# artpixls/ART

Measured on AMD Instinct MI355X. Metric: megapixels/sec end-to-end (AMaZE+FTblockDN+tone), 45 MP Bayer, higher is better.
Workload: dtype f32; 1 GPU; AMaZE + getImage/matrix + ImProcFunctions::denoise (chroma noise-curve map, FTblockDN wavelet shrinkage luma 40 / chroma 15 / gamma 1.7 + DCT detail recovery 50) + exposure 0.3 EV + tone curve STD, 8192x5464 Bayer RGGB fp32, 1 frame per GPU per step (BASELINE configs[2]); frame=8192x5464, lanes_per_gpu=1, parallelism=frame-per-gpu x1, completion_records=1, completion_via=single process

## Files before the change

### art_amd/csrc/artgpu_api.hip

```cpp
#include <hip/hip_runtime.h>
#include <dlfcn.h>
#include <cmath>
#include <cstdio>
#include <cstdarg>
#include <cstring>
#include <new>
#include <string>
#include <thread>
#include <vector>
#include <algorithm>

#include "../../include/artgpu.h"
#include "kernels.h"

using namespace artgpu;

struct artgpu_ctx {
    int device = 0;
    hipStream_t stream = nullptr;
    hipStream_t aux = nullptr;
    hipEvent_t aux_ev[2] = {nullptr, nullptr};
    hipStream_t dn_stream[1] = {nullptr};
    hipEvent_t dn_ev[2] = {nullptr, nullptr};
    const float *gam_tab = nullptr; float gam_key[6] = {};
    int opt_lut_lds = 1;
    int opt_dn_streams = 0;
    int ccalc_nonneg = 0;
    int opt_dn_fused = 1;
    std::string err;
    int *fs_diag = nullptr;
    int opt_dn_debug_stall = -1;
    long opt_dn_wait_ms = 0;
    long long batch_px = 0;
    int dn_form = -1, dn_form_streak = 0;
    float *arena = nullptr;
    size_t arena_bytes = 0;
    static constexpr int NSTAGE = 8;
    float *stage[NSTAGE] = {};
    size_t stage_bytes[NSTAGE] = {};
    static constexpr int NPOOL = 64;
    float *pool[NPOOL] = {};
    size_t pool_bytes[NPOOL] = {};
    std::vector<artgpu_ctx *> lanes;
    int batch_lanes = 1;
    int frames_in_flight = 1;
    bool owns_stream = false;
    hipStream_t io_up = nullptr, io_down = nullptr;
    hipEvent_t io_ev[8] = {};
    int *io_host = nullptr;
    int io_host_cap = 0;
// ... 375 lines not shown
        const size_t nfixed = (((size_t)ctx->amz_nstream + (1 + ctx->amz_narena) + (1 + ctx->amz_narena + ctx->amz_nstream) + 3) / 4) * 4;
        int v = 0;
        HIPCHK(ctx, hipMemcpy(&v, reinterpret_cast<int *>(ctx->amz_lists) + nfixed + 4 + 2 * (size_t)ctx->amz_nstream + (n[13] - '0'), sizeof(int), hipMemcpyDeviceToHost));
        *value = v;
        return ARTGPU_OK;
    }
    return fail(ctx, ARTGPU_EINVAL, "get_option: unknown option '%s'", name);
}

int artgpu_set_option(artgpu_ctx *ctx, const char *name, long value)
{
    if (!ctx || !name) return ARTGPU_EINVAL;
    const std::string n(name);
    if (n == "amaze_path") { if (value < 0 || value > 1) return fail(ctx, ARTGPU_EINVAL, "amaze_path: 0 or 1"); ctx->opt_amaze_path = (int)value; }
    else if (n == "amaze_split") ctx->opt_amaze_split = value != 0;
    else if (n == "amaze_overlap") ctx->opt_amaze_overlap = value != 0;
    else if (n == "amaze_grid") { if (value < 0) return fail(ctx, ARTGPU_EINVAL, "amaze_grid: >= 0"); ctx->opt_amaze_grid = (int)value; }
    else if (n == "amaze_zero_mask") ctx->opt_amaze_zero_mask = value;
    else if (n == "amaze_zero_frame") ctx->opt_amaze_zero_frame = (int)value;
    else if (n == "amaze_poison") ctx->opt_amaze_poison = (int)value;
    else if (n == "roctx") ctx->opt_roctx = value != 0;
    else if (n == "dn_streams") ctx->opt_dn_streams = value != 0;
    else if (n == "dn_fused") ctx->opt_dn_fused = (int)value;
    else if (n == "dn_debug_stall") ctx->opt_dn_debug_stall = (int)value;
    else if (n == "dn_wait_ms") ctx->opt_dn_wait_ms = value < 0 ? 0 : value;
    else if (n == "lut_lds") ctx->opt_lut_lds = value != 0;
    else if (n == "cu_reserve") { if (value < 0 || value > 4096) return fail(ctx, ARTGPU_EINVAL, "cu_reserve: 0 .. 4096"); ctx->cu_reserve = (int)value; }
    else if (n == "io_direct") { if (value < -1 || value > 4096) return fail(ctx, ARTGPU_EINVAL, "io_direct: -1 (automatic), 0 .. 4096 workgroups"); ctx->opt_io_direct = (int)value; }
    else if (n == "rcd_rows") { if (value != 4 && value != 8) return fail(ctx, ARTGPU_EINVAL, "rcd_rows: 4 or 8"); ctx->opt_rcd_rows = (int)value; }
    else return fail(ctx, ARTGPU_EINVAL, "set_option: unknown option '%s'", name);
    return ARTGPU_OK;
}

int artgpu_set_progress_callback(artgpu_ctx *ctx, artgpu_progress_fn fn, void *user)
{
    if (!ctx) return ARTGPU_EINVAL;
    ctx->progress_fn = fn;
    ctx->progress_user = user;
    return ARTGPU_OK;
}

int artgpu_enable_timing(artgpu_ctx *ctx, int enable)
{
    if (!ctx) return ARTGPU_EINVAL;
    ctx->timing = enable != 0;
    return ARTGPU_OK;
// ... 391 lines not shown
    a.tail_kind = ctx->curve_tail_kind == ARTGPU_CURVE_TAIL_HOST ? 0 : ctx->curve_tail_kind; a.tail_y = ctx->curve_tail_y; a.tail_pc = ctx->curve_tail_pc;
    if (lut65536) {
        if ((rc = upload_curve(ctx, lut65536))) return rc;
        a.lut = ctx->lut;
    }
    a.no_lds_lut = !ctx->opt_lut_lds; a.cu_reserve = ctx->cu_reserve;
    HIPCHK(ctx, launch_tone_std(a, ctx->stream));
    return unbind_rgb(ctx, image, &d);
}

}

struct artgpu_wavelet {
    int w = 0, h = 0, w2 = 0, h2 = 0, nlevels = 0;
    float *bands = nullptr;
    float *lowpass[2] = {nullptr, nullptr};
    int cur = 0;
    size_t n = 0;
    float *band(int l, int dir) const { return bands + ((size_t)l * 3 + (dir - 1)) * n; }
};

namespace {
int wavelet_skip(int level) { return level <= 1 ? 1 : 1 << (level - 1); }
}

extern "C" {

int artgpu_wavelet_decompose(artgpu_ctx *ctx, const artgpu_plane *src, int maxlvl, artgpu_wavelet **out)
{
    if (!ctx) return ARTGPU_EINVAL;
    if (!plane_ok(src) || !out || maxlvl < 1 || maxlvl > 9) return fail(ctx, ARTGPU_EINVAL, "wavelet_decompose: bad arguments");
    *out = nullptr;
    const int w = src->w, h = src->h, w2 = (w + 1) / 2, h2 = (h + 1) / 2;
    if ((w2 < h2 ? w2 : h2) < 2 * wavelet_skip(maxlvl - 1) || w < 8 || h < 8)
        return fail(ctx, ARTGPU_EUNSUPPORTED, "wavelet_decompose: %dx%d too small for %d levels", w, h, maxlvl);
    HIPCHK(ctx, hipSetDevice(ctx->device));
    const float *dsrc = src->p;
    size_t sstride = (size_t)(src->row_stride_bytes / 4);
    if (!src->on_device) {
        int rc = ensure(ctx, &ctx->stage[0], &ctx->stage_bytes[0], (size_t)w * h * 4);
        if (rc) return rc;
        HIPCHK(ctx, hipMemcpy2DAsync(ctx->stage[0], (size_t)w * 4, src->p, (size_t)src->row_stride_bytes, (size_t)w * 4, h, hipMemcpyHostToDevice, ctx->stream));
        dsrc = ctx->stage[0];
        sstride = w;
    }
    artgpu_wavelet *wv = new (std::nothrow) artgpu_wavelet;
    if (!wv) return fail(ctx, ARTGPU_ENOMEM, "wavelet_decompose: out of host memory");
    wv->w = w; wv->h = h; wv->w2 = w2; wv->h2 = h2; wv->nlevels = maxlvl; wv->n = (size_t)w2 * h2;
    hipError_t e = hipMalloc(reinterpret_cast<void **>(&wv->bands), (size_t)maxlvl * 3 * wv->n * sizeof(float));
    if (e == hipSuccess) e = hipMalloc(reinterpret_cast<void **>(&wv->lowpass[0]), wv->n * sizeof(float));
    if (e == hipSuccess) e = hipMalloc(reinterpret_cast<void **>(&wv->lowpass[1]), wv->n * sizeof(float));
    if (e != hipSuccess) {
        artgpu_wavelet_free(ctx, wv);
        return fail(ctx, ARTGPU_ENOMEM, "wavelet_decompose: hipMalloc failed: %s", hipGetErrorString(e));
    }
    WaveArgs a = {};
    a.w = w; a.h = h; a.w2 = w2; a.h2 = h2;
    for (int l = 0; l < maxlvl; ++l) {
        a.b1 = wv->band(l, 1); a.b2 = wv->band(l, 2); a.b3 = wv->band(l, 3);
        hipError_t le;
        if (l == 0) {
            a.src = dsrc; a.src_stride = sstride; a.lo = wv->lowpass[0];
            wv->cur = 0;
            le = launch_wavelet_analysis0(a, ctx->stream);
        } else {
            a.src = wv->lowpass[wv->cur]; a.lo = wv->lowpass[wv->cur ^ 1]; a.skip = wavelet_skip(l);
            le = launch_wavelet_haar_analysis(a, ctx->stream);
            wv->cur ^= 1;
        }
        if (le != hipSuccess) {
            artgpu_wavelet_free(ctx, wv);
            return fail(ctx, ARTGPU_EHIP, "wavelet_decompose: launch failed: %s", hipGetErrorString(le));
        }
    }
    if (!src->on_device) {
        const hipError_t se = hipStreamSynchronize(ctx->stream);
        if (se != hipSuccess) {
            artgpu_wavelet_free(ctx, wv);
            return fail(ctx, ARTGPU_EHIP, "wavelet_decompose: %s", hipGetErrorString(se));
        }
    }
    *out = wv;
    return ARTGPU_OK;
}

int artgpu_wavelet_info(const artgpu_wavelet *wv, int32_t *w2, int32_t *h2, int32_t *nlevels)
{
    if (!wv) return ARTGPU_EINVAL;
    if (w2) *w2 = wv->w2;
    if (h2) *h2 = wv->h2;
    if (nlevels) *nlevels = wv->nlevels;
    return ARTGPU_OK;
}

int artgpu_wavelet_get_band(artgpu_ctx *ctx, const artgpu_wavelet *wv, int level, int dir, float *dst, int on_device)
{
// ... 13 lines not shown
    HIPCHK(ctx, hipSetDevice(ctx->device));
    float *p = dir == 0 ? wv->lowpass[wv->cur] : wv->band(level, dir);
    HIPCHK(ctx, hipMemcpyAsync(p, src, wv->n * sizeof(float), on_device ? hipMemcpyDeviceToDevice : hipMemcpyHostToDevice, ctx->stream));
    if (!on_device) HIPCHK(ctx, hipStreamSynchronize(ctx->stream));
    return ARTGPU_OK;
}

int artgpu_wavelet_reconstruct(artgpu_ctx *ctx, artgpu_wavelet *wv, artgpu_plane *dst, float blend)
{
    if (!ctx) return ARTGPU_EINVAL;
    if (!wv || !plane_ok(dst) || dst->w != wv->w || dst->h != wv->h) return fail(ctx, ARTGPU_EINVAL, "wavelet_reconstruct: bad arguments");
    HIPCHK(ctx, hipSetDevice(ctx->device));
    float *ddst = dst->p;
    size_t dstride = (size_t)(dst->row_stride_bytes / 4);
    if (!dst->on_device) {
        int rc = ensure(ctx, &ctx->stage[0], &ctx->stage_bytes[0], (size_t)wv->w * wv->h * 4);
        if (rc) return rc;
        HIPCHK(ctx, hipMemcpy2DAsync(ctx->stage[0], (size_t)wv->w * 4, dst->p, (size_t)dst->row_stride_bytes, (size_t)wv->w * 4, wv->h, hipMemcpyHostToDevice, ctx->stream));
        ddst = ctx->stage[0];
        dstride = wv->w;
    }
    WaveArgs a = {};
    a.w = wv->w; a.h = wv->h; a.w2 = wv->w2; a.h2 = wv->h2; a.blend = blend;
    for (int l = wv->nlevels - 1; l > 0; --l) {
        a.src = wv->lowpass[wv->cur]; a.lo = wv->lowpass[wv->cur ^ 1];
        a.b1 = wv->band(l, 1); a.b2 = wv->band(l, 2); a.b3 = wv->band(l, 3); a.skip = wavelet_skip(l);
        HIPCHK(ctx, launch_wavelet_haar_synthesis(a, ctx->stream));
        wv->cur ^= 1;
    }
    a.src = wv->lowpass[wv->cur];
    a.b1 = wv->band(0, 1); a.b2 = wv->band(0, 2); a.b3 = wv->band(0, 3);
    a.dst = ddst; a.dst_stride = dstride;
    HIPCHK(ctx, launch_wavelet_synthesis0(a, ctx->stream));
    if (!dst->on_device) {
        HIPCHK(ctx, hipMemcpy2DAsync(dst->p, (size_t)dst->row_stride_bytes, ddst, (size_t)wv->w * 4, (size_t)wv->w * 4, wv->h, hipMemcpyDeviceToHost, ctx->stream));
        HIPCHK(ctx, hipStreamSynchronize(ctx->stream));
    }
    return ARTGPU_OK;
}

int artgpu_wavelet_free(artgpu_ctx *ctx, artgpu_wavelet *wv)
{
    if (!wv) return ARTGPU_EINVAL;
    if (ctx) { (void)hipSetDevice(ctx->device); (void)hipStreamSynchronize(ctx->stream); }
    if (wv->bands) (void)hipFree(wv->bands);
    if (wv->lowpass[0]) (void)hipFree(wv->lowpass[0]);
    if (wv->lowpass[1]) (void)hipFree(wv->lowpass[1]);
    delete wv;
    return ARTGPU_OK;
}

}

namespace {

enum { P_L = 0, P_A, P_B, P_LBANDS, P_LLOW0, P_LLOW1, P_CBANDS, P_CLOW0, P_CLOW1, P_SF, P_TMP, P_HISTO, P_MAD, P_GAM, P_CCALC, P_LIN, P_BLOCKS, P_DTAB, P_CCMAP, P_CACHEF, P_PQ, P_XCBRT, P_GAUSS64, P_DMASK, P_LABTABS, P_PIPE_R, P_PIPE_G, P_PIPE_B, P_DNINFO, P_BATCH, P_DCTTAB, P_CBANDS2, P_CLOW0_2, P_CLOW1_2, P_SF_A, P_SF_B, P_HISTO_A, P_HISTO_B, P_RGBCURVES, P_FUSED, P_LBANDS2,
       P_IO_IN0, P_IO_IN1, P_IO_CFA, P_IO_IMG0, P_IO_IMG1, P_IO_IMG2, P_IO_IMG3, P_IO_IMG4, P_IO_IMG5, P_IO_OUT0, P_IO_OUT1, P_IO_FLAGS,
       P_NSLOTS };
static_assert(P_NSLOTS <= artgpu_ctx::NPOOL, "grow artgpu_ctx::pool");

struct DevDecomp {
    float *bands, *low[2];
    int cur, nlevels, w, h, w2, h2;
    size_t n;
    float *band(int l, int dir) const { return bands + ((size_t)l * 3 + (dir - 1)) * n; }
};

int decompose_dev(artgpu_ctx *ctx, DevDecomp &d, const float *src, hipStream_t st = nullptr)
{
    if (!st) st = ctx->stream;
    WaveArgs a = {};
    a.w = d.w; a.h = d.h; a.w2 = d.w2; a.h2 = d.h2;
    for (int l = 0; l < d.nlevels; ++l) {
        a.b1 = d.band(l, 1); a.b2 = d.band(l, 2); a.b3 = d.band(l, 3);
        if (l == 0) {
            a.src = src; a.src_stride = d.w; a.lo = d.low[0]; d.cur = 0;
            HIPCHK(ctx, launch_wavelet_analysis0(a, st));
        } else {
            a.src = d.low[d.cur]; a.lo = d.low[d.cur ^ 1]; a.skip = wavelet_skip(l);
            HIPCHK(ctx, launch_wavelet_haar_analysis(a, st));
            d.cur ^= 1;
        }
    }
    return ARTGPU_OK;
}

int reconstruct_dev(artgpu_ctx *ctx, DevDecomp &d, float *dst, hipStream_t st = nullptr)
{
    if (!st) st = ctx->stream;
    WaveArgs a = {};
    a.w = d.w; a.h = d.h; a.w2 = d.w2; a.h2 = d.h2; a.blend = 1.f;
    for (int l = d.nlevels - 1; l > 0; --l) {
        a.src = d.low[d.cur]; a.lo = d.low[d.cur ^ 1];
        a.b1 = d.band(l, 1); a.b2 = d.band(l, 2); a.b3 = d.band(l, 3); a.skip = wavelet_skip(l);
        HIPCHK(ctx, launch_wavelet_haar_synthesis(a, st));
        d.cur ^= 1;
    }
    a.src = d.low[d.cur];
    a.b1 = d.band(0, 1); a.b2 = d.band(0, 2); a.b3 = d.band(0, 3);
    a.dst = dst; a.dst_stride = d.w;
    HIPCHK(ctx, launch_wavelet_synthesis0(a, st));
    return ARTGPU_OK;
}

int pool_get(artgpu_ctx *ctx, int slot, size_t bytes, float **out)
{
    int rc = ensure(ctx, &ctx->pool[slot], &ctx->pool_bytes[slot], bytes);
    *out = ctx->pool[slot];
    return rc;
}

}

extern "C" {

namespace {
int detail_mask_dev(artgpu_ctx *ctx, const float *src, size_t src_stride, float *mask, int W, int H,
                    float scaling, float threshold, float ceiling, float factor, float blur, float *scratch);
}

int artgpu_wavelet_mad(artgpu_ctx *ctx, const artgpu_wavelet *wv, float *mad_sqr)
{
    if (!ctx) return ARTGPU_EINVAL;
    if (!wv || !mad_sqr) return fail(ctx, ARTGPU_EINVAL, "wavelet_mad: null argument");
    if (wv->n > 0x7fffffff) return fail(ctx, ARTGPU_EUNSUPPORTED, "wavelet_mad: band larger than an int holds (MadRgb's datalen is an int)");
// ... 166 lines not shown
    px.igam_lds_lo = 8000;
    if (lab_mode) {
        float *tabs;
        const bool fresh = ctx->pool[P_LABTABS] == nullptr;
        if ((rc = pool_get(ctx, P_LABTABS, 4 * 65536 * 4, &tabs))) return rc;
        if (fresh) {
            std::vector<float> host(4 * 65536);
            build_cachef(host.data()); build_cachefy(host.data() + 65536);
            build_denoise_gamma_tabs(host.data() + 2 * 65536, host.data() + 3 * 65536);
            hipError_t e = hipMemcpyAsync(tabs, host.data(), host.size() * 4, hipMemcpyHostToDevice, sL);
            if (e == hipSuccess) e = hipStreamSynchronize(sL);
            if (e != hipSuccess) {
                (void)hipFree(ctx->pool[P_LABTABS]); ctx->pool[P_LABTABS] = nullptr; ctx->pool_bytes[P_LABTABS] = 0;
                return fail(ctx, ARTGPU_EHIP, "rgb_denoise: upload of the Lab tables failed: %s", hipGetErrorString(e));
            }
        }
        px.lab_mode = 1;
        px.cachef = tabs; px.cachefy = tabs + 65536; px.dn_gamma = tabs + 2 * 65536; px.dn_igamma = tabs + 3 * 65536;
        for (int k = 0; k < 9; ++k) { px.wpi[k] = ws[k]; px.iws[k] = iws[k]; }
    }
    px.realred = realred; px.realblue = realblue; px.qhighFactor = aggressive ? 1.f / static_cast<float>(0.9) : 1.0f;
    HIPCHK(ctx, launch_rgb2yuv(px, sL));

    if ((rc = decompose_dev(ctx, Ld, L, sL))) return rc;
    if (!merged_mad) HIPCHK(ctx, launch_mad(Ld.bands, n2, nsub, reinterpret_cast<int *>(histo_fc[0]), madL, sL));

    auto fused_pass = [&](bool ab, const float *cin, float *cout, const float *cL, const float *mL, const float *mab, int lev0, int nb,
                          float nv_const, float noisevar_ab) -> int {
        FusedShrinkArgs fa = {};
        if (ab) { fa.coefC = cout; fa.nL = 0; fa.nsub_ch = nb; }
        else { fa.coef = cin; fa.coef_out = cout; fa.nL = nb; }
        fa.coefL = cL; fa.n = n2; fa.w = w2; fa.h = h2;
        fa.madL = mL; fa.madab = mab;
        fa.noisevar = ccalc_dev; fa.noisevar_nonneg = ctx->ccalc_nonneg; fa.noisevar_const = nv_const; fa.noisevar_scale = maxNoiseVarab; fa.noisevar_ab[0] = fa.noisevar_ab[1] = noisevar_ab;
        fa.useNoiseCCurve = useNoiseCCurve ? 1 : 0;
        for (int l = 0; l < 10; ++l) fa.rad[l] = bl0.rad[l];
        fa.level0 = lev0; fa.nsub = nb; fa.diag = ctx->fs_diag; fa.wait_ticks = (long long)ctx->opt_dn_wait_ms * 100000LL; fa.stall_band = ctx->opt_dn_debug_stall < 0 ? -1 : ctx->opt_dn_debug_stall >> 16; fa.stall_strip = ctx->opt_dn_debug_stall < 0 ? -1 : ctx->opt_dn_debug_stall & 0xffff;
        HIPCHK(ctx, launch_shrink_blur(fa, fused_scratch, sL));
        return ARTGPU_OK;
    };

    float noisevar_abc[2];
    auto chroma_front = [&](int ch) -> int {
        DevDecomp &Cd = Cdd[ch];
        float *sf = sfc[1 + ch], *tmp = tmpc[1 + ch], *madab = mad + 32 * (1 + ch);
        int *histo = reinterpret_cast<int *>(histo_fc[1 + ch]);
        float noisevar_ab = ch == 0 ? noisevarab_r : noisevarab_b;
        if (autoch && noisevar_ab <= 0.001f) noisevar_ab = 0.02f;
        noisevar_abc[ch] = noisevar_ab;
        int rc2;
        if ((rc2 = decompose_dev(ctx, Cd, ch == 0 ? A : B, sL))) return rc2;
        if (aggressive && noisevar_ab > 0.001f) {
            HIPCHK(ctx, launch_mad(Cd.bands, n2, nsub, histo, madab, sL));
            ShrinkArgs sa = {};
            sa.n = n2; sa.noisevar = ccalc_dev; sa.noisevar_scale = maxNoiseVarab; sa.noisevar_ab = noisevar_ab; sa.useNoiseCCurve = useNoiseCCurve ? 1 : 0;
            const size_t top = (size_t)(nsub - 3) * n2;
            sa.coef = Cd.bands + top; sa.coefL = Ld.bands + top; sa.sfave = sf; sa.madL = madL + (nsub - 3); sa.madab = madab + (nsub - 3);
            if (fused) {
                if ((rc2 = fused_pass(true, Cd.bands + top, Cd.bands + top, Ld.bands + top, madL + (nsub - 3), madab + (nsub - 3), levwav - 1, 3, 0.f, noisevar_ab))) return rc2;
            } else {
                HIPCHK(ctx, launch_shrink_sf(sa, 3, true, sL));
                BlurArgs bt = bl0;
                bt.level0 = levwav - 1;
                bt.src = sf; bt.dst = tmp;
                HIPCHK(ctx, launch_hblur(bt, 3, sL));
                bt.src = tmp; bt.sfave = sf; bt.coef = Cd.bands + top;
                HIPCHK(ctx, launch_vblur_combine(bt, 3, sL));
            }
            if (nsub > 3) {
                sa.coef = Cd.bands; sa.coefL = Ld.bands; sa.madL = madL; sa.madab = madab;
                HIPCHK(ctx, launch_bishrink_AB(sa, nsub - 3, sL));
            }
        }
        if (noisevar_ab > 0.001f && !merged_mad) {
// ... 22 lines not shown
                HIPCHK(ctx, launch_hblur(bl, nsub, sL));
                bl.src = tmp; bl.sfave = sf; bl.coef = Cd.bands;
                HIPCHK(ctx, launch_vblur_combine(bl, nsub, sL));
            }
        }
        if (nresi || highresi) {
            float host[32];
            HIPCHK(ctx, launch_mad(Cd.bands, n2, nsub, histo, madab, sL));
            HIPCHK(ctx, hipMemcpyAsync(host, madab, (size_t)nsub * sizeof(float), hipMemcpyDeviceToHost, sL));
            HIPCHK(ctx, hipStreamSynchronize(sL));
            float resid = 0.f, maxresid = 0.f;
            for (int k = 0; k < nsub; ++k) {
                resid += host[k];
                if (host[k] > maxresid) maxresid = host[k];
            }
            if (ch == 0) { chresidtemp = resid; chmaxresidtemp = maxresid; }
            else {
                float chresid = resid + chresidtemp, chmaxresid = maxresid + chmaxresidtemp;
                chresid = std::sqrt(chresid / (6 * (levwav)));
                if (highresi) *highresi = chresid + 0.66f * (std::sqrt(chmaxresid) - chresid);
                if (nresi) *nresi = chresid;
            }
        }
        return reconstruct_dev(ctx, Cd, ch == 0 ? A : B, sL);
    };

    float *Lout = L;
    auto luma = [&](hipStream_t sd) -> int {
        if (!denoiseLuminance) return ARTGPU_OK;
        int rc2;
        const int nsubL = 3 * (levwav < 5 ? levwav : 5);
        float *sf = sfc[0], *tmp = tmpc[0];
        BlurArgs bl = bl0;
        ShrinkArgs sa = {};
        sa.coef = Ld.bands; sa.sfave = sf; sa.n = n2; sa.madL = madL; sa.noisevar = nullptr; sa.noisevar_const = noisevarL;
        DevDecomp Lrec = Ld;
        if (merged) Lrec.bands = Lbands2;
        for (int rep = aggressive ? 0 : 1; rep < 2 && !merged; ++rep) {
            if (fused) {
                float *dstb = Lbands2 ? Lbands2 : Ld.bands;
                if ((rc2 = fused_pass(false, Lrec.bands, dstb, nullptr, madL, nullptr, 0, nsubL, noisevarL, 0.f))) return rc2;
                Lrec.bands = dstb;
            } else {
                HIPCHK(ctx, launch_shrink_sf(sa, nsubL, false, sL));
                bl.src = sf; bl.dst = tmp;
                HIPCHK(ctx, launch_hblur(bl, nsubL, sL));
                bl.src = tmp; bl.sfave = sf; bl.coef = Ld.bands;
                HIPCHK(ctx, launch_vblur_combine(bl, nsubL, sL));
            }
        }
        if (Lrec.bands != Ld.bands && nsubL < nsub)
            HIPCHK(ctx, hipMemcpyAsync(Lrec.bands + (size_t)nsubL * n2, Ld.bands + (size_t)nsubL * n2, (size_t)(nsub - nsubL) * n2 * 4, hipMemcpyDeviceToDevice, sL));
        if (do_detail) {
            if ((rc2 = pool_get(ctx, P_LIN, n * 4, &Lout))) return rc2;
        }
        Lrec.cur = Ld.cur;
        if ((rc2 = reconstruct_dev(ctx, Lrec, Lout, sL))) return rc2;
        if (do_detail) {
            float *Lin = L;
            DetailArgs da = {};
            da.w = w; da.h = h;
            da.numblox_W = (int)std::ceil(((float)w) / 25) + 2;
            da.numblox_H = (int)std::ceil(((float)h) / 25) + 2;
            const float params_Ldetail = std::min(float(p->luminance_detail), 99.9f);
            auto compute_detail = [](float dd) -> float { const float t = static_cast<float>((100. - dd) * (100. - dd) + 50. * (100. - dd)) * 64 * 0.5f; return t * t; };
            da.detail_hi = compute_detail(params_Ldetail);
            da.detail_lo = compute_detail(0.f);
            { const int br = int(3 / scale); da.blur_rad = br > 1 ? br : 1; }
            float *dtab;
            const bool fresh_dtab = ctx->pool[P_DCTTAB] == nullptr;
            if ((rc2 = pool_get(ctx, P_DCTTAB, 4 * 4096 * 4, &dtab))) return rc2;
            if ((rc2 = pool_get(ctx, P_BLOCKS, (size_t)da.numblox_W * da.numblox_H * 4096 * 4, &da.blocks))) return rc2;
            if (fresh_dtab) {
                std::vector<float> host(4 * 4096);
                float *tm_in = host.data(), *tm_out = tm_in + 4096, *ct = tm_out + 4096, *ctt = ct + 4096;
                const float epsilon = 0.001f / (64 * 64);
                const int border = 4;
                for (int i = 0; i < 64; ++i) {
                    const float i1 = std::abs((i > 32 ? i - 64 + 1 : i));
                    const float vmask = (i1 < border ? (float)0 + (std::sin((M_PI * i1) / (2 * border)) * std::sin((M_PI * i1) / (2 * border))) : 1.0f);
// ... 1398 lines not shown
        if (rc) return rc;
        c->batch_px = 0;
    }
    if (px > c->batch_px) c->batch_px = px;
    return ARTGPU_OK;
}

int batch_prepare_lanes(artgpu_ctx *ctx, int L)
{
    HIPCHK(ctx, hipSetDevice(ctx->device));
    while ((int)ctx->lanes.size() < L - 1) {
        artgpu_ctx *peer = nullptr;
        int rc = artgpu_create(ctx->device, &peer);
        if (rc) return fail(ctx, rc, "batch_run: cannot create lane %d", (int)ctx->lanes.size() + 1);
        if (hipStreamCreateWithFlags(&peer->stream, hipStreamNonBlocking) != hipSuccess) { (void)artgpu_destroy(peer); return fail(ctx, ARTGPU_EHIP, "batch_run: stream"); }
        peer->owns_stream = true;
        ctx->lanes.push_back(peer);
    }
    for (artgpu_ctx *peer : ctx->lanes) {
        peer->curve_tail_kind = ctx->curve_tail_kind; peer->curve_tail_y = ctx->curve_tail_y; peer->curve_tail_pc = ctx->curve_tail_pc;
        peer->opt_amaze_path = ctx->opt_amaze_path; peer->opt_amaze_split = ctx->opt_amaze_split; peer->opt_amaze_overlap = ctx->opt_amaze_overlap; peer->opt_amaze_grid = ctx->opt_amaze_grid;
        peer->opt_amaze_zero_mask = ctx->opt_amaze_zero_mask; peer->opt_amaze_zero_frame = ctx->opt_amaze_zero_frame; peer->opt_amaze_poison = ctx->opt_amaze_poison;
        peer->opt_rcd_rows = ctx->opt_rcd_rows; peer->opt_roctx = ctx->opt_roctx; peer->opt_lut_lds = ctx->opt_lut_lds; peer->opt_dn_streams = ctx->opt_dn_streams; peer->opt_dn_fused = ctx->opt_dn_fused;
        peer->opt_dn_wait_ms = ctx->opt_dn_wait_ms; peer->opt_dn_debug_stall = ctx->opt_dn_debug_stall; peer->opt_io_direct = ctx->opt_io_direct;
        peer->progress_fn = ctx->progress_fn; peer->progress_user = ctx->progress_user;
        peer->frames_in_flight = L;
    }
    ctx->frames_in_flight = L;
    return ARTGPU_OK;
}
struct InFlightReset { artgpu_ctx *c; ~InFlightReset() { c->frames_in_flight = 1; for (artgpu_ctx *p : c->lanes) p->frames_in_flight = 1; } };

extern "C++" {
template <typename F>
int batch_on_lanes(artgpu_ctx *ctx, int L, F work)
{
    std::vector<int> rcs(L, ARTGPU_OK);
    std::vector<artgpu_ctx *> cs(L, ctx);
    for (int k = 1; k < L; ++k) cs[k] = ctx->lanes[k - 1];
    std::vector<std::thread> threads;
    for (int k = 1; k < L; ++k) threads.emplace_back([&rcs, &work, &cs, k]() { rcs[k] = work(cs[k], k); });
    rcs[0] = work(ctx, 0);
    for (std::thread &t : threads) t.join();
    for (int k = 0; k < L; ++k)
        if (rcs[k]) return fail(ctx, rcs[k], "batch_run: lane %d: %s", k, k == 0 ? ctx->err.c_str() : cs[k]->err.c_str());
    return ARTGPU_OK;
// ... 249 lines not shown
```

### art_amd/csrc/kernels.h

```cpp
#pragma once
#include <hip/hip_runtime.h>
#include "paramcurve.h"
#include <vector>
#include <stddef.h>
#include <stdint.h>
#include <mutex>
#include <set>
#include <utility>

inline hipError_t dyn_lds_once(const void *fn, int bytes)
{
    static std::mutex m;
    static std::set<std::pair<const void *, int>> done;
    int dev = 0;
    hipError_t e = hipGetDevice(&dev);
    if (e != hipSuccess) return e;
    std::lock_guard<std::mutex> lk(m);
    if (done.count({fn, dev})) return hipSuccess;
    e = hipFuncSetAttribute(fn, hipFuncAttributeMaxDynamicSharedMemorySize, bytes);
    if (e == hipSuccess) done.insert({fn, dev});
    return e;
}

inline bool device_block_fits(int lds_bytes, int threads)
// ... 273 lines not shown
    int cu_reserve;
};
hipError_t launch_neutral_hues(const NeutralArgs &a, hipStream_t s);
hipError_t launch_tone_neutral(const NeutralArgs &a, hipStream_t s);
void build_pq_luts(float *pq65536, float *pq_inv65536);
void dninfo_band_stats(const float *mad_a, const float *mad_b, int nbands, bool aggressive, float out[6]);
void dninfo_reduce(const float info[9][16], bool aggressive, float ch_M[9], float max_r[9], float max_b[9], float out3[3]);

struct WaveArgs {
    const float *src;
    size_t src_stride;
    float *lo;
    float *b1, *b2, *b3;
    float *dst;
    size_t dst_stride;
    int w, h, w2, h2;
    int skip;
    float blend;
};
hipError_t launch_wavelet_analysis0(const WaveArgs &a, hipStream_t s);
hipError_t launch_wavelet_haar_analysis(const WaveArgs &a, hipStream_t s);
hipError_t launch_wavelet_haar_synthesis(const WaveArgs &a, hipStream_t s);
hipError_t launch_wavelet_synthesis0(const WaveArgs &a, hipStream_t s);

struct GetImageFuse {
    int on;
    const float *src[3];
    size_t stride;
    int sx1, sy1;
    float mul[3];
    int do_clip, has_mat;
    double mat[9];
};
struct DnPixArgs {
    GetImageFuse gi;
    float exp_scale, exp_black;
    int exp_on;
    float *rgb[3];
    size_t stride;
    float *L, *A, *B;
    int w, h;
    float gain, newGain;
    float gam, gamthresh, gamslope, igam, igamthresh, igamslope;
    const float *gamcurve, *igamcurve;
    float ws1[3];
    float realred, realblue, qhighFactor;
// ... 164 lines not shown
```

### art_amd/csrc/wavelet.hip

```cpp
#include <hip/hip_runtime.h>
#include "devmath.h"
#include "kernels.h"

namespace artgpu {

namespace {
__constant__ float DAUB_LO[6] = {0.f, 0.f, 0.34150635f, 0.59150635f, 0.15849365f, -0.091506351f};
__constant__ float DAUB_HI[6] = {-0.091506351f, -0.15849365f, 0.59150635f, -0.34150635f, 0.f, 0.f};
__constant__ float SYN_LO[6] = {-0.091506351f, 0.15849365f, 0.59150635f, 0.34150635f, 0.f, 0.f};
__constant__ float SYN_HI[6] = {0.f, 0.f, -0.34150635f, 0.59150635f, -0.15849365f, -0.091506351f};
__device__ __forceinline__ int clampi(int v, int lo, int hi) { return v < lo ? lo : (v > hi ? hi : v); }

#ifndef A0_TW_
#define A0_TW_ 64
#endif
#ifndef A0_TH_
#ifdef A0_PLAIN
#define A0_TH_ 16
#else
#define A0_TH_ 32
#endif
#endif
constexpr int A0_TW = A0_TW_, A0_TH = A0_TH_;
constexpr int A0_LW = 2 * A0_TW + 6;
// ... 222 lines not shown
        const int t = threadIdx.x + n * 256;
        const int rr = t / S0_TW, cc = t - rr * S0_TW;
        const int i = min(r0 + rr, h - 1), k = min(c0 + cc, w - 1);
        dv[n] = use_old ? a.dst[(size_t)i * a.dst_stride + k] : 0.f;
    }
#pragma unroll
    for (int n = 0; n < NIT; ++n) {
        const int t = threadIdx.x + n * 256;
        const int rr = t / S0_TW, cc = t - rr * S0_TW;
        const int i = r0 + rr, k = c0 + cc;
        if (i >= h || k >= w) continue;
        const int i_src = (i + shift) / 2;
        float tot = 0.f;
#pragma unroll
        for (int l = 0; l < 3; ++l) {
            const int lr = clampi(i_src - l, 0, h2 - 1) - srow0;
            tot += (flo[l] * tLo[lr][cc] + fhi[l] * tHi[lr][cc]);
        }
        const size_t o = (size_t)i * a.dst_stride + k;
        a.dst[o] = dv[n] * srcFactor + a.blend * 4.f * tot;
    }
}

hipError_t launch_wavelet_analysis0(const WaveArgs &a, hipStream_t s)
{
    dim3 grid((a.w2 + A0_TW - 1) / A0_TW, (a.h2 + A0_TH - 1) / A0_TH);
    hipLaunchKernelGGL(wavelet_analysis0_kernel, grid, dim3(256), 0, s, a);
    return hipGetLastError();
}
static int flat_grid(long long n) { long long g = (n + 255) / 256; return (int)(g < 16384 ? g : 16384); }
hipError_t launch_wavelet_haar_analysis(const WaveArgs &a, hipStream_t s)
{
    hipLaunchKernelGGL(wavelet_haar_analysis_kernel, dim3(flat_grid((long long)a.w2 * a.h2)), dim3(256), 0, s, a);
    return hipGetLastError();
}
hipError_t launch_wavelet_haar_synthesis(const WaveArgs &a, hipStream_t s)
{
    hipLaunchKernelGGL(wavelet_haar_synthesis_kernel, dim3(flat_grid((long long)a.w2 * a.h2)), dim3(256), 0, s, a);
    return hipGetLastError();
}
hipError_t launch_wavelet_synthesis0(const WaveArgs &a, hipStream_t s)
{
    dim3 grid((a.w + S0_TW - 1) / S0_TW, (a.h + S0_TH - 1) / S0_TH);
    hipLaunchKernelGGL(wavelet_synthesis0_kernel, grid, dim3(256), 0, s, a);
    return hipGetLastError();
}
// ... 3 lines not shown
```

Before: 4428 MP/s.

## Fuse multiple Haar wavelet levels into streaming row-sweep kernels across channels

```diff
diff --git a/art_amd/csrc/artgpu_api.hip b/art_amd/csrc/artgpu_api.hip
--- a/art_amd/csrc/artgpu_api.hip
+++ b/art_amd/csrc/artgpu_api.hip
@@ -26,6 +26,8 @@
     int opt_lut_lds = 1;
     int opt_dn_streams = 0;
     int ccalc_nonneg = 0;
+    int opt_wav_stream = 1;
+    int opt_wav_seg = 0;
     int opt_dn_fused = 1;
     std::string err;
     int *fs_diag = nullptr;
@@ -447,6 +449,8 @@
     else if (n == "roctx") ctx->opt_roctx = value != 0;
     else if (n == "dn_streams") ctx->opt_dn_streams = value != 0;
     else if (n == "dn_fused") ctx->opt_dn_fused = (int)value;
+    else if (n == "wav_stream") ctx->opt_wav_stream = value != 0;
+    else if (n == "wav_seg") { if (value < 0 || value > 65536) return fail(ctx, ARTGPU_EINVAL, "wav_seg: 0 (automatic) .. 65536 rows"); ctx->opt_wav_seg = (int)value; }
     else if (n == "dn_debug_stall") ctx->opt_dn_debug_stall = (int)value;
     else if (n == "dn_wait_ms") ctx->opt_dn_wait_ms = value < 0 ? 0 : value;
     else if (n == "lut_lds") ctx->opt_lut_lds = value != 0;
@@ -884,6 +888,63 @@
 
 namespace {
 int wavelet_skip(int level) { return level <= 1 ? 1 : 1 << (level - 1); }
+
+struct HaarChan {
+    float *bands, *low[2];
+    int *cur;
+    float *band(int l, int dir, size_t n) const { return bands + ((size_t)l * 3 + (dir - 1)) * n; }
+};
+
+hipError_t haar_analysis_levels(const artgpu_ctx *ctx, const HaarChan *c, int nch, int w2, int h2, size_t n, int nlevels, hipStream_t st)
+{
+    int l = 1;
+    const int nl = nlevels - 1 < WAVE_STREAM_MAXL ? nlevels - 1 : WAVE_STREAM_MAXL;
+    if (ctx->opt_wav_stream && wavelet_haar_stream_supported(w2, h2, nl)) {
+        WaveStreamArgs a = {};
+        a.n = n; a.w = w2; a.h = h2; a.nl = nl; a.seg_h = ctx->opt_wav_seg;
+        for (int k = 0; k < nch; ++k) { a.src[k] = c[k].low[*c[k].cur]; a.lo[k] = c[k].low[*c[k].cur ^ 1]; a.bands[k] = c[k].bands; }
+        const hipError_t e = launch_wavelet_haar_stream_analysis(a, nch, st);
+        if (e != hipSuccess) return e;
+        for (int k = 0; k < nch; ++k) *c[k].cur ^= 1;
+        l = nl + 1;
+    }
+    for (int k = 0; k < nch; ++k)
+        for (int m = l; m < nlevels; ++m) {
+            WaveArgs a = {};
+            a.w2 = w2; a.h2 = h2; a.skip = wavelet_skip(m);
+            a.src = c[k].low[*c[k].cur]; a.lo = c[k].low[*c[k].cur ^ 1];
+            a.b1 = c[k].band(m, 1, n); a.b2 = c[k].band(m, 2, n); a.b3 = c[k].band(m, 3, n);
+            const hipError_t e = launch_wavelet_haar_analysis(a, st);
+            if (e != hipSuccess) return e;
+            *c[k].cur ^= 1;
+        }
+    return hipSuccess;
+}
+
+hipError_t haar_synthesis_levels(const artgpu_ctx *ctx, const HaarChan *c, int nch, int w2, int h2, size_t n, int nlevels, hipStream_t st)
+{
+    const int nl = nlevels - 1 < WAVE_STREAM_MAXL ? nlevels - 1 : WAVE_STREAM_MAXL;
+    const bool streamed = ctx->opt_wav_stream && wavelet_haar_stream_supported(w2, h2, nl);
+    for (int k = 0; k < nch; ++k)
+        for (int m = nlevels - 1; m > (streamed ? nl : 0); --m) {
+            WaveArgs a = {};
+            a.w2 = w2; a.h2 = h2; a.skip = wavelet_skip(m);
+            a.src = c[k].low[*c[k].cur]; a.lo = c[k].low[*c[k].cur ^ 1];
+            a.b1 = c[k].band(m, 1, n); a.b2 = c[k].band(m, 2, n); a.b3 = c[k].band(m, 3, n);
+            const hipError_t e = launch_wavelet_haar_synthesis(a, st);
+            if (e != hipSuccess) return e;
+            *c[k].cur ^= 1;
+        }
+    if (streamed) {
+        WaveStreamArgs a = {};
+        a.n = n; a.w = w2; a.h = h2; a.nl = nl; a.seg_h = ctx->opt_wav_seg;
+        for (int k = 0; k < nch; ++k) { a.src[k] = c[k].low[*c[k].cur]; a.lo[k] = c[k].low[*c[k].cur ^ 1]; a.bands[k] = c[k].bands; }
+        const hipError_t e = launch_wavelet_haar_stream_synthesis(a, nch, st);
+        if (e != hipSuccess) return e;
+        for (int k = 0; k < nch; ++k) *c[k].cur ^= 1;
+    }
+    return hipSuccess;
+}
 }
 
 extern "C" {
@@ -918,22 +979,17 @@
     }
     WaveArgs a = {};
     a.w = w; a.h = h; a.w2 = w2; a.h2 = h2;
-    for (int l = 0; l < maxlvl; ++l) {
-        a.b1 = wv->band(l, 1); a.b2 = wv->band(l, 2); a.b3 = wv->band(l, 3);
-        hipError_t le;
-        if (l == 0) {
-            a.src = dsrc; a.src_stride = sstride; a.lo = wv->lowpass[0];
-            wv->cur = 0;
-            le = launch_wavelet_analysis0(a, ctx->stream);
-        } else {
-            a.src = wv->lowpass[wv->cur]; a.lo = wv->lowpass[wv->cur ^ 1]; a.skip = wavelet_skip(l);
-            le = launch_wavelet_haar_analysis(a, ctx->stream);
-            wv->cur ^= 1;
-        }
-        if (le != hipSuccess) {
-            artgpu_wavelet_free(ctx, wv);
-            return fail(ctx, ARTGPU_EHIP, "wavelet_decompose: launch failed: %s", hipGetErrorString(le));
-        }
+    a.b1 = wv->band(0, 1); a.b2 = wv->band(0, 2); a.b3 = wv->band(0, 3);
+    a.src = dsrc; a.src_stride = sstride; a.lo = wv->lowpass[0];
+    wv->cur = 0;
+    hipError_t le = launch_wavelet_analysis0(a, ctx->stream);
+    if (le == hipSuccess) {
+        const HaarChan c = {wv->bands, {wv->lowpass[0], wv->lowpass[1]}, &wv->cur};
+        le = haar_analysis_levels(ctx, &c, 1, w2, h2, wv->n, maxlvl, ctx->stream);
+    }
+    if (le != hipSuccess) {
+        artgpu_wavelet_free(ctx, wv);
+        return fail(ctx, ARTGPU_EHIP, "wavelet_decompose: launch failed: %s", hipGetErrorString(le));
     }
     if (!src->on_device) {
         const hipError_t se = hipStreamSynchronize(ctx->stream);
@@ -993,11 +1049,9 @@
     }
     WaveArgs a = {};
     a.w = wv->w; a.h = wv->h; a.w2 = wv->w2; a.h2 = wv->h2; a.blend = blend;
-    for (int l = wv->nlevels - 1; l > 0; --l) {
-        a.src = wv->lowpass[wv->cur]; a.lo = wv->lowpass[wv->cur ^ 1];
-        a.b1 = wv->band(l, 1); a.b2 = wv->band(l, 2); a.b3 = wv->band(l, 3); a.skip = wavelet_skip(l);
-        HIPCHK(ctx, launch_wavelet_haar_synthesis(a, ctx->stream));
-        wv->cur ^= 1;
+    {
+        const HaarChan c = {wv->bands, {wv->lowpass[0], wv->lowpass[1]}, &wv->cur};
+        HIPCHK(ctx, haar_synthesis_levels(ctx, &c, 1, wv->w2, wv->h2, wv->n, wv->nlevels, ctx->stream));
     }
     a.src = wv->lowpass[wv->cur];
     a.b1 = wv->band(0, 1); a.b2 = wv->band(0, 2); a.b3 = wv->band(0, 3);
@@ -1037,41 +1091,51 @@
     float *band(int l, int dir) const { return bands + ((size_t)l * 3 + (dir - 1)) * n; }
 };
 
+int decompose_multi(artgpu_ctx *ctx, DevDecomp *const *ds, const float *const *srcs, int nch, hipStream_t st)
+{
+    HaarChan c[3];
+    for (int k = 0; k < nch; ++k) {
+        DevDecomp &d = *ds[k];
+        WaveArgs a = {};
+        a.w = d.w; a.h = d.h; a.w2 = d.w2; a.h2 = d.h2;
+        a.b1 = d.band(0, 1); a.b2 = d.band(0, 2); a.b3 = d.band(0, 3);
+        a.src = srcs[k]; a.src_stride = d.w; a.lo = d.low[0]; d.cur = 0;
+        HIPCHK(ctx, launch_wavelet_analysis0(a, st));
+        c[k] = HaarChan{d.bands, {d.low[0], d.low[1]}, &d.cur};
+    }
+    const DevDecomp &d0 = *ds[0];
+    HIPCHK(ctx, haar_analysis_levels(ctx, c, nch, d0.w2, d0.h2, d0.n, d0.nlevels, st));
+    return ARTGPU_OK;
+}
+
 int decompose_dev(artgpu_ctx *ctx, DevDecomp &d, const float *src, hipStream_t st = nullptr)
 {
-    if (!st) st = ctx->stream;
-    WaveArgs a = {};
-    a.w = d.w; a.h = d.h; a.w2 = d.w2; a.h2 = d.h2;
-    for (int l = 0; l < d.nlevels; ++l) {
-        a.b1 = d.band(l, 1); a.b2 = d.band(l, 2); a.b3 = d.band(l, 3);
-        if (l == 0) {
-            a.src = src; a.src_stride = d.w; a.lo = d.low[0]; d.cur = 0;
-            HIPCHK(ctx, launch_wavelet_analysis0(a, st));
-        } else {
-            a.src = d.low[d.cur]; a.lo = d.low[d.cur ^ 1]; a.skip = wavelet_skip(l);
-            HIPCHK(ctx, launch_wavelet_haar_analysis(a, st));
-            d.cur ^= 1;
-        }
+    DevDecomp *ds[1] = {&d};
+    return decompose_multi(ctx, ds, &src, 1, st ? st : ctx->stream);
+}
+
+int reconstruct_multi(artgpu_ctx *ctx, DevDecomp *const *ds, float *const *dsts, int nch, hipStream_t st)
+{
+    HaarChan c[3];
+    for (int k = 0; k < nch; ++k) c[k] = HaarChan{ds[k]->bands, {ds[k]->low[0], ds[k]->low[1]}, &ds[k]->cur};
+    const DevDecomp &d0 = *ds[0];
+    HIPCHK(ctx, haar_synthesis_levels(ctx, c, nch, d0.w2, d0.h2, d0.n, d0.nlevels, st));
+    for (int k = 0; k < nch; ++k) {
+        DevDecomp &d = *ds[k];
+        WaveArgs a = {};
+        a.w = d.w; a.h = d.h; a.w2 = d.w2; a.h2 = d.h2; a.blend = 1.f;
+        a.src = d.low[d.cur];
+        a.b1 = d.band(0, 1); a.b2 = d.band(0, 2); a.b3 = d.band(0, 3);
+        a.dst = dsts[k]; a.dst_stride = d.w;
+        HIPCHK(ctx, launch_wavelet_synthesis0(a, st));
     }
     return ARTGPU_OK;
 }
 
 int reconstruct_dev(artgpu_ctx *ctx, DevDecomp &d, float *dst, hipStream_t st = nullptr)
 {
-    if (!st) st = ctx->stream;
-    WaveArgs a = {};
-    a.w = d.w; a.h = d.h; a.w2 = d.w2; a.h2 = d.h2; a.blend = 1.f;
-    for (int l = d.nlevels - 1; l > 0; --l) {
-        a.src = d.low[d.cur]; a.lo = d.low[d.cur ^ 1];
-        a.b1 = d.band(l, 1); a.b2 = d.band(l, 2); a.b3 = d.band(l, 3); a.skip = wavelet_skip(l);
-        HIPCHK(ctx, launch_wavelet_haar_synthesis(a, st));
-        d.cur ^= 1;
-    }
-    a.src = d.low[d.cur];
-    a.b1 = d.band(0, 1); a.b2 = d.band(0, 2); a.b3 = d.band(0, 3);
-    a.dst = dst; a.dst_stride = d.w;
-    HIPCHK(ctx, launch_wavelet_synthesis0(a, st));
-    return ARTGPU_OK;
+    DevDecomp *ds[1] = {&d};
+    return reconstruct_multi(ctx, ds, &dst, 1, st ? st : ctx->stream);
 }
 
 int pool_get(artgpu_ctx *ctx, int slot, size_t bytes, float **out)
@@ -1284,7 +1348,11 @@
     px.realred = realred; px.realblue = realblue; px.qhighFactor = aggressive ? 1.f / static_cast<float>(0.9) : 1.0f;
     HIPCHK(ctx, launch_rgb2yuv(px, sL));
 
-    if ((rc = decompose_dev(ctx, Ld, L, sL))) return rc;
+    if (merged) {
+        DevDecomp *ds[3] = {&Ld, &Cdd[0], &Cdd[1]};
+        const float *srcs[3] = {L, A, B};
+        if ((rc = decompose_multi(ctx, ds, srcs, 3, sL))) return rc;
+    } else if ((rc = decompose_dev(ctx, Ld, L, sL))) return rc;
     if (!merged_mad) HIPCHK(ctx, launch_mad(Ld.bands, n2, nsub, reinterpret_cast<int *>(histo_fc[0]), madL, sL));
 
     auto fused_pass = [&](bool ab, const float *cin, float *cout, const float *cL, const float *mL, const float *mab, int lev0, int nb,
@@ -1311,7 +1379,7 @@
         if (autoch && noisevar_ab <= 0.001f) noisevar_ab = 0.02f;
         noisevar_abc[ch] = noisevar_ab;
         int rc2;
-        if ((rc2 = decompose_dev(ctx, Cd, ch == 0 ? A : B, sL))) return rc2;
+        if (!merged && (rc2 = decompose_dev(ctx, Cd, ch == 0 ? A : B, sL))) return rc2;
         if (aggressive && noisevar_ab > 0.001f) {
             HIPCHK(ctx, launch_mad(Cd.bands, n2, nsub, histo, madab, sL));
             ShrinkArgs sa = {};
@@ -1380,7 +1448,7 @@
                 if (nresi) *nresi = chresid;
             }
         }
-        return reconstruct_dev(ctx, Cd, ch == 0 ? A : B, sL);
+        return merged ? ARTGPU_OK : reconstruct_dev(ctx, Cd, ch == 0 ? A : B, sL);
     };
 
     float *Lout = L;
@@ -1413,7 +1481,11 @@
             if ((rc2 = pool_get(ctx, P_LIN, n * 4, &Lout))) return rc2;
         }
         Lrec.cur = Ld.cur;
-        if ((rc2 = reconstruct_dev(ctx, Lrec, Lout, sL))) return rc2;
+        if (merged) {
+            DevDecomp *ds[3] = {&Lrec, &Cdd[0], &Cdd[1]};
+            float *dsts[3] = {Lout, A, B};
+            if ((rc2 = reconstruct_multi(ctx, ds, dsts, 3, sL))) return rc2;
+        } else if ((rc2 = reconstruct_dev(ctx, Lrec, Lout, sL))) return rc2;
         if (do_detail) {
             float *Lin = L;
             DetailArgs da = {};
@@ -2858,6 +2930,7 @@
         peer->opt_amaze_path = ctx->opt_amaze_path; peer->opt_amaze_split = ctx->opt_amaze_split; peer->opt_amaze_overlap = ctx->opt_amaze_overlap; peer->opt_amaze_grid = ctx->opt_amaze_grid;
         peer->opt_amaze_zero_mask = ctx->opt_amaze_zero_mask; peer->opt_amaze_zero_frame = ctx->opt_amaze_zero_frame; peer->opt_amaze_poison = ctx->opt_amaze_poison;
         peer->opt_rcd_rows = ctx->opt_rcd_rows; peer->opt_roctx = ctx->opt_roctx; peer->opt_lut_lds = ctx->opt_lut_lds; peer->opt_dn_streams = ctx->opt_dn_streams; peer->opt_dn_fused = ctx->opt_dn_fused;
+        peer->opt_wav_stream = ctx->opt_wav_stream; peer->opt_wav_seg = ctx->opt_wav_seg;
         peer->opt_dn_wait_ms = ctx->opt_dn_wait_ms; peer->opt_dn_debug_stall = ctx->opt_dn_debug_stall; peer->opt_io_direct = ctx->opt_io_direct;
         peer->progress_fn = ctx->progress_fn; peer->progress_user = ctx->progress_user;
         peer->frames_in_flight = L;
diff --git a/art_amd/csrc/kernels.h b/art_amd/csrc/kernels.h
--- a/art_amd/csrc/kernels.h
+++ b/art_amd/csrc/kernels.h
@@ -319,6 +319,19 @@
 hipError_t launch_wavelet_haar_analysis(const WaveArgs &a, hipStream_t s);
 hipError_t launch_wavelet_haar_synthesis(const WaveArgs &a, hipStream_t s);
 hipError_t launch_wavelet_synthesis0(const WaveArgs &a, hipStream_t s);
+struct WaveStreamArgs {
+    const float *src[3];
+    float *lo[3];
+    float *bands[3];
+    size_t n;
+    int w, h;
+    int nl;
+    int seg_h;
+};
+constexpr int WAVE_STREAM_MAXL = 4;
+bool wavelet_haar_stream_supported(int w2, int h2, int nl);
+hipError_t launch_wavelet_haar_stream_analysis(const WaveStreamArgs &a, int nch, hipStream_t s);
+hipError_t launch_wavelet_haar_stream_synthesis(const WaveStreamArgs &a, int nch, hipStream_t s);
 
 struct GetImageFuse {
     int on;
diff --git a/art_amd/csrc/wavelet.hip b/art_amd/csrc/wavelet.hip
--- a/art_amd/csrc/wavelet.hip
+++ b/art_amd/csrc/wavelet.hip
@@ -1,4 +1,5 @@
 #include <hip/hip_runtime.h>
+#include <algorithm>
 #include "devmath.h"
 #include "kernels.h"
 
@@ -268,6 +269,211 @@
     }
 }
 
+namespace {
+constexpr int WS_T = 256;
+__device__ __forceinline__ void ws_lds_barrier()
+{
+    __builtin_amdgcn_fence(__ATOMIC_RELEASE, "workgroup", "local");
+    __builtin_amdgcn_s_barrier();
+    __builtin_amdgcn_fence(__ATOMIC_ACQUIRE, "workgroup", "local");
+}
+constexpr int ring_a_off(int k) { int o = 0; for (int j = 1; j < k; ++j) o += (1 << j) + 1; return o; }
+constexpr int ring_s_off(int k) { int o = 0; for (int j = 1; j < k; ++j) o += (1 << (j - 1)) + 1; return o; }
+constexpr unsigned WS_DROP = 0x80000000u;
+__device__ __forceinline__ __amdgpu_buffer_rsrc_t ws_rsrc(float *p, size_t floats)
+{
+    return __builtin_amdgcn_make_buffer_rsrc(p, 0, (int)(floats * 4), 0x00020000);
+}
+__device__ __forceinline__ void ws_store(__amdgpu_buffer_rsrc_t r, unsigned off_bytes, float v)
+{
+    __builtin_amdgcn_raw_buffer_store_b32(__float_as_uint(v), r, (int)off_bytes, 0, 0);
+}
+}
+
+template <int NL>
+__global__ void __launch_bounds__(WS_T) wavelet_haar_analysis_stream_kernel(WaveStreamArgs a)
+{
+    constexpr int REACH = (1 << NL) - 1, SW = WS_T - REACH, LAG = REACH + NL, PF = 4, RT = ring_a_off(NL + 1);
+    __shared__ float tl[NL][2][WS_T], th[NL][2][WS_T];
+    const int w = a.w, h = a.h, ch = blockIdx.z, tid = threadIdx.x;
+    const float *src = a.src[ch];
+    const size_t n = a.n;
+    const __amdgpu_buffer_rsrc_t rb = ws_rsrc(a.bands[ch], 3 * (NL + 1) * n), rl = ws_rsrc(a.lo[ch], n);
+    const int c0 = blockIdx.x * SW, c1 = min(c0 + SW, w);
+    const int r0 = blockIdx.y * a.seg_h, r1 = min(r0 + a.seg_h, h);
+    const int xlo = min(c0, w - (1 << NL)), ylo = min(r0, h - (1 << NL));
+    const int x = xlo + tid, xc = min(x, w - 1);
+    const bool xst = x >= c0 && x < c1;
+    int nb[NL];
+#pragma unroll
+    for (int k = 0; k < NL; ++k) { const int s = 1 << k; nb[k] = min(max(x < w - s ? tid + s : tid - s, 0), WS_T - 1); }
+    const int yend = r1 - 1 + LAG;
+    const int ylast = min(h, r1 + REACH) - 1;
+    float ring[RT];
+#pragma unroll
+    for (int i = 0; i < RT; ++i) ring[i] = 0.f;
+    float pf[PF];
+#pragma unroll
+    for (int j = 0; j < PF; ++j) pf[j] = src[(size_t)min(ylo + j, ylast) * w + xc];
+    for (int yb = ylo; yb <= yend; yb += PF) {
+#pragma unroll
+        for (int j = 0; j < PF; ++j) {
+            const int y = yb + j;
+            float carry = pf[j];
+            pf[j] = src[(size_t)min(y + PF, ylast) * w + xc];
+            const int par = y & 1;
+            int hrow = y;
+#pragma unroll
+            for (int k = 1; k <= NL; ++k) {
+                const int s = 1 << (k - 1), off = ring_a_off(k);
+#pragma unroll
+                for (int i = 2 * s; i > 0; --i) ring[off + i] = ring[off + i - 1];
+                ring[off] = carry;
+                const int vr = hrow - s;
+                const float s0 = ring[off + s], s1 = vr < h - s ? ring[off] : ring[off + 2 * s];
+                tl[k - 1][par][tid] = 0.25f * (s0 + s1);
+                th[k - 1][par][tid] = 0.25f * (s0 - s1);
+                const int hr = vr - 1;
+                const float t0 = tl[k - 1][par ^ 1][tid], t1 = tl[k - 1][par ^ 1][nb[k - 1]];
+                const float u0 = th[k - 1][par ^ 1][tid], u1 = th[k - 1][par ^ 1][nb[k - 1]];
+                const float lo = t0 + t1;
+                const bool st = xst && hr >= r0 && hr < r1;
+                const unsigned o = (unsigned)hr * w + x, ob = (unsigned)(3 * k) * (unsigned)n + o;
+                ws_store(rb, st ? ob * 4 : WS_DROP, t0 - t1);
+                ws_store(rb, st ? (ob + (unsigned)n) * 4 : WS_DROP, u0 + u1);
+                ws_store(rb, st ? (ob + 2 * (unsigned)n) * 4 : WS_DROP, u0 - u1);
+                if (k == NL) ws_store(rl, st ? o * 4 : WS_DROP, lo);
+                carry = lo;
+                hrow = hr;
+            }
+            ws_lds_barrier();
+        }
+    }
+}
+
+template <int NL>
+__global__ void __launch_bounds__(WS_T) wavelet_haar_synthesis_stream_kernel(WaveStreamArgs a)
+{
+    constexpr int REACH = (1 << NL) - 1, SW = WS_T - REACH, PF = 2, NLD = 1 + 3 * NL, RT = ring_s_off(NL + 1);
+    __shared__ float st[NL][2][4][WS_T];
+    const int w = a.w, h = a.h, ch = blockIdx.z, tid = threadIdx.x;
+    const float *src = a.src[ch], *bands = a.bands[ch];
+    const size_t n = a.n;
+    const __amdgpu_buffer_rsrc_t rl = ws_rsrc(a.lo[ch], n);
+    const int c0 = blockIdx.x * SW, c1 = min(c0 + SW, w);
+    const int r0 = blockIdx.y * a.seg_h, r1 = min(r0 + a.seg_h, h);
+    const int xlo = max(c0 - REACH, 0), ylo = max(r0 - REACH, 0);
+    const int x = xlo + tid, xc = min(x, w - 1);
+    const bool xst = x >= c0 && x < c1;
+    int jp[NL];
+    bool fj[NL];
+#pragma unroll
+    for (int k = 0; k < NL; ++k) { const int s = 1 << k; fj[k] = x < s; jp[k] = fj[k] ? tid : max(tid - s, 0); }
+    const int yend = r1 - 1 + NL;
+    auto load = [&](float (&v)[NLD], int y) {
+        v[0] = src[(size_t)min(max(y, 0), r1 - 1) * w + xc];
+#pragma unroll
+        for (int m = 1; m <= NL; ++m) {
+            const size_t o = (size_t)min(max(y - (NL - m), 0), r1 - 1) * w + xc;
+            const float *b = bands + (size_t)(3 * m) * n;
+            v[3 * m - 2] = b[o]; v[3 * m - 1] = b[n + o]; v[3 * m] = b[2 * n + o];
+        }
+    };
+    float rlo[RT], rhi[RT];
+#pragma unroll
+    for (int i = 0; i < RT; ++i) rlo[i] = rhi[i] = 0.f;
+    float pf[PF][NLD];
+#pragma unroll
+    for (int j = 0; j < PF; ++j) load(pf[j], ylo + j);
+    for (int yb = ylo; yb <= yend; yb += PF) {
+#pragma unroll
+        for (int j = 0; j < PF; ++j) {
+            const int y = yb + j;
+            const int par = y & 1;
+            st[NL - 1][par][0][tid] = pf[j][0];
+#pragma unroll
+            for (int m = 1; m <= NL; ++m) {
+                st[m - 1][par][1][tid] = pf[j][3 * m - 2]; st[m - 1][par][2][tid] = pf[j][3 * m - 1]; st[m - 1][par][3][tid] = pf[j][3 * m];
+            }
+            load(pf[j], y + PF);
+#pragma unroll
+            for (int k = NL; k >= 1; --k) {
+                const int s = 1 << (k - 1), off = ring_s_off(k);
+                const int q = y - 1 - (NL - k);
+                const int p = jp[k - 1];
+                const float (*S)[WS_T] = st[k - 1][par ^ 1];
+                const float tLo = haar_syn(S[0][tid], S[1][tid], S[0][p], S[1][p], fj[k - 1]);
+                const float tHi = haar_syn(S[2][tid], S[3][tid], S[2][p], S[3][p], fj[k - 1]);
+#pragma unroll
+                for (int i = s; i > 0; --i) { rlo[off + i] = rlo[off + i - 1]; rhi[off + i] = rhi[off + i - 1]; }
+                rlo[off] = tLo; rhi[off] = tHi;
+                const float r = q < s ? tLo + tHi : 0.5f * (tLo + tHi + rlo[off + s] - rhi[off + s]);
+                if (k > 1) st[k - 2][par][0][tid] = r;
+                else ws_store(rl, xst && q >= r0 && q < r1 ? ((unsigned)q * w + x) * 4 : WS_DROP, r);
+            }
+            ws_lds_barrier();
+        }
+    }
+}
+
+bool wavelet_haar_stream_supported(int w2, int h2, int nl)
+{
+    return nl >= 1 && nl <= WAVE_STREAM_MAXL && w2 >= (1 << nl) && h2 >= (1 << nl) && (double)w2 * h2 * 4 * 3 * (nl + 1) < (double)WS_DROP;
+}
+static int ws_resident(const void *kernel)
+{
+    int dev = 0, cus = 0, per_cu = 0;
+    if (hipGetDevice(&dev) != hipSuccess || hipDeviceGetAttribute(&cus, hipDeviceAttributeMultiprocessorCount, dev) != hipSuccess ||
+        hipOccupancyMaxActiveBlocksPerMultiprocessor(&per_cu, kernel, WS_T, 0) != hipSuccess || cus * per_cu <= 0) {
+        (void)hipGetLastError();
+        return 1024;
+    }
+    return cus * per_cu;
+}
+static int ws_grid(const WaveStreamArgs &a, int nch, const void *kernel, dim3 &grid)
+{
+    const int sw = WS_T - ((1 << a.nl) - 1), strips = (a.w + sw - 1) / sw;
+    int seg = a.seg_h;
+    if (seg <= 0) {
+        const int nseg = std::max(1, ws_resident(kernel) / (strips * nch));
+        seg = std::max((a.h + nseg - 1) / nseg, 32);
+    }
+    grid = dim3(strips, (a.h + seg - 1) / seg, nch);
+    return seg;
+}
+hipError_t launch_wavelet_haar_stream_analysis(const WaveStreamArgs &a0, int nch, hipStream_t s)
+{
+    if (nch < 1 || nch > 3 || !wavelet_haar_stream_supported(a0.w, a0.h, a0.nl)) return hipErrorInvalidValue;
+    WaveStreamArgs a = a0;
+    dim3 grid;
+    const void *k[4] = {(const void *)wavelet_haar_analysis_stream_kernel<1>, (const void *)wavelet_haar_analysis_stream_kernel<2>,
+                         (const void *)wavelet_haar_analysis_stream_kernel<3>, (const void *)wavelet_haar_analysis_stream_kernel<4>};
+    a.seg_h = ws_grid(a0, nch, k[a.nl - 1], grid);
+    switch (a.nl) {
+    case 1: hipLaunchKernelGGL(wavelet_haar_analysis_stream_kernel<1>, grid, dim3(WS_T), 0, s, a); break;
+    case 2: hipLaunchKernelGGL(wavelet_haar_analysis_stream_kernel<2>, grid, dim3(WS_T), 0, s, a); break;
+    case 3: hipLaunchKernelGGL(wavelet_haar_analysis_stream_kernel<3>, grid, dim3(WS_T), 0, s, a); break;
+    default: hipLaunchKernelGGL(wavelet_haar_analysis_stream_kernel<4>, grid, dim3(WS_T), 0, s, a); break;
+    }
+    return hipGetLastError();
+}
+hipError_t launch_wavelet_haar_stream_synthesis(const WaveStreamArgs &a0, int nch, hipStream_t s)
+{
+    if (nch < 1 || nch > 3 || !wavelet_haar_stream_supported(a0.w, a0.h, a0.nl)) return hipErrorInvalidValue;
+    WaveStreamArgs a = a0;
+    dim3 grid;
+    const void *k[4] = {(const void *)wavelet_haar_synthesis_stream_kernel<1>, (const void *)wavelet_haar_synthesis_stream_kernel<2>,
+                         (const void *)wavelet_haar_synthesis_stream_kernel<3>, (const void *)wavelet_haar_synthesis_stream_kernel<4>};
+    a.seg_h = ws_grid(a0, nch, k[a.nl - 1], grid);
+    switch (a.nl) {
+    case 1: hipLaunchKernelGGL(wavelet_haar_synthesis_stream_kernel<1>, grid, dim3(WS_T), 0, s, a); break;
+    case 2: hipLaunchKernelGGL(wavelet_haar_synthesis_stream_kernel<2>, grid, dim3(WS_T), 0, s, a); break;
+    case 3: hipLaunchKernelGGL(wavelet_haar_synthesis_stream_kernel<3>, grid, dim3(WS_T), 0, s, a); break;
+    default: hipLaunchKernelGGL(wavelet_haar_synthesis_stream_kernel<4>, grid, dim3(WS_T), 0, s, a); break;
+    }
+    return hipGetLastError();
+}
+
 hipError_t launch_wavelet_analysis0(const WaveArgs &a, hipStream_t s)
 {
     dim3 grid((a.w2 + A0_TW - 1) / A0_TW, (a.h2 + A0_TH - 1) / A0_TH);
```

Measured after the change: 4472 MP/s, median of 6. About the same (+1.0%).
